# esteinig/sketchy

Hardware: AMD Instinct MI355X
Metric: reads/sec streamed (s=10000,k=16,40k-genome ref) (higher is better)
Workload: dtype u64

## Files before the change

sketchy_amd/csrc/skx_capi.hip:

```cpp
#include <dlfcn.h>
#include <hip/hip_runtime.h>
#include <rccl/rccl.h>

#include <unistd.h>

#include <algorithm>
#include <atomic>
#include <chrono>
#include <cmath>
#include <condition_variable>
#include <cstdarg>
#include <cstdio>
#include <cstdlib>
#include <cstring>
#include <mutex>
#include <string>
#include <thread>
#include <unordered_map>
#include <vector>

#include "sketchy_hip.h"
#include "skx_common.hpp"
#include "skx_kernels.hpp"

// ... 918 lines not shown
    hipEvent_t ev_pairq[2] = {nullptr, nullptr};
    bool pairq_pending[2] = {false, false};
    bool packed = false;
    u32 top_k = 0, max_reads = 0, sk_stride = 0;
    u64 max_bases = 0;
    u32 pcap = 0;
    u32 qcap = 0;
    u64* d_qd = nullptr;
    u32 *d_qrow = nullptr, *d_sslot = nullptr, *d_qinfo = nullptr, *d_qloc = nullptr, *d_cls_bsum = nullptr;
    u32* d_nd_hs = nullptr;
    u32* h_lcount = nullptr;
    u32 lcount_seq = 0, lcount_seen = 0, lcount_floor = 0;
    u32* h_nq_sink = nullptr;
    u32* h_nd = nullptr;
    u32 *d_rowcnt = nullptr;
    u32 *d_gain = nullptr;
    u32 *d_gain_s = nullptr;
    u32 *d_candslot = nullptr;
    u32 *d_candmask = nullptr;
    uint2 *d_lrow = nullptr;
    u32 *d_nlrow = nullptr, *d_gain_l = nullptr, *d_cbase = nullptr, *d_cwl = nullptr, *d_ncwl = nullptr;
    u64 *d_cw = nullptr;
    u64 *d_inb = nullptr, *d_hit = nullptr;
    skx::LongRows long_rows() const { return skx::LongRows{d_lrow, d_nlrow, qcap + 128, d_inb, ref->n_lw}; }
    bool use_pat = false;
    u32 *d_hist = nullptr, *d_nprow = nullptr;
    u64* d_pcw = nullptr;
    u32 npat_pad = 0;
    skx::PatRows pat_rows() const { return skx::PatRows{d_hist, npat_pad, d_gain_l, d_nprow}; }
    skx::RareIndex rare_index() const {
        skx::RareIndex ri = ref->rare_index();
        if (!use_pat) { ri.prec = nullptr; ri.n_pat = 0; }
        if (!static_dense) { ri.qs = nullptr; ri.n_sd = 0; }
        return ri;
    }
    u32 *d_cbad = nullptr, *d_nqc = nullptr;
    u32 *d_spc_g0 = nullptr, *d_spc_grp = nullptr;
    u32 n_pad_c = 0, n_grp_c = 0, cand_seq = 0;
    struct PassSet {
        u64 *tab = nullptr;
        u32 *cand = nullptr;
        u64 *tabc = nullptr;
        u32 *ncand = nullptr;
        u32 *mode = nullptr, *any_full = nullptr, *nqc_total = nullptr;
        u64 *mc = nullptr;
        u64 *mqc = nullptr;
        u64 *rowany_c = nullptr;
        u32 *grp_any_c = nullptr;
        u32 *smap = nullptr;
        u32 *pair_qc = nullptr;
        u32 *nd = nullptr;
        u32 *h_pub = nullptr;
    } ps[2];
    struct PassChains {
        bool pending = false, ranked = false, has_cand = false, update_table = false, forced_full = false, legacy = false;
        SubPass subs[kGroupMax];
        int n_sub = 0, b = 0, slot = 0;
        u32 P = 0, nq_rows = 0, seq = 0;
        u64 nq_est = 0;
// ... 646 lines not shown
        SCHK(hipMalloc(&st->d_cbad, 64));
        SCHK(hipMalloc(&st->d_nqc, skx::pass_counter_bytes()));
        std::vector<u32> g0c(n_sp), grpc(st->n_grp_c);
        for (u32 i = 0; i < n_sp; ++i) g0c[i] = i * cap;
        for (u32 i = 0; i < st->n_grp_c; ++i) grpc[i] = i / (cap / (skx::kRankWords * 64));
        SCHK(hipMalloc(&st->d_spc_g0, (size_t)n_sp * 4));
        SCHK(hipMalloc(&st->d_spc_grp, (size_t)st->n_grp_c * 4));
        SCHK(hipMemcpy(st->d_spc_g0, g0c.data(), (size_t)n_sp * 4, hipMemcpyHostToDevice));
        SCHK(hipMemcpy(st->d_spc_grp, grpc.data(), (size_t)st->n_grp_c * 4, hipMemcpyHostToDevice));
        for (auto& q : st->ps) {
            SCHK(hipMalloc(&q.tab, (size_t)(nb + 1) * n_pad * 8));
            SCHK(hipMalloc(&q.cand, (size_t)nb * st->n_pad_c * 4));
            SCHK(hipMalloc(&q.tabc, (size_t)nb * st->n_pad_c * 8));
            SCHK(hipMalloc(&q.ncand, (size_t)nb * n_sp * 4));
            SCHK(hipMalloc(&q.mode, 64)); SCHK(hipMalloc(&q.any_full, 64)); SCHK(hipMalloc(&q.nqc_total, 64));
            SCHK(hipMemset(q.any_full, 0, 64));
            SCHK(hipMalloc(&q.mc, (size_t)nb * (rows_c / 64) * st->n_pad_c * 8));
            SCHK(hipMalloc(&q.mqc, (size_t)nb * st->n_grp_c * rows_c * skx::kRankWords * 8));
            SCHK(hipMalloc(&q.rowany_c, (size_t)nb * st->n_grp_c * (rows_c / 64) * 8));
            SCHK(hipMalloc(&q.grp_any_c, (size_t)nb * st->n_grp_c * 4 + 64));
            SCHK(hipMalloc(&q.smap, (size_t)nb * ((size_t)st->qcap + 128) * 4));
            SCHK(hipMalloc(&q.pair_qc, (size_t)st->pcap * 4));
            SCHK(hipMalloc(&q.nd, 64));
            SCHK(hipMemset(q.nd, 0, 64));
            SCHK(hipHostMalloc((void**)&q.h_pub, 32 * 4, hipHostMallocCoherent));
            memset(q.h_pub, 0, 32 * 4);
        }
    }
    SCHK(hipDeviceSynchronize());
#undef SCHK
// ... 115 lines not shown
        const u32 any[4] = {skx::mq_any_stride(), 0xFFFFFFFFu, skx::mq_any_stride(), 0xFFFFFFFFu};
        e = hipMemcpy(st->d_mqext, any, sizeof(any), hipMemcpyHostToDevice);
    }
    if (e == hipSuccess && mint) e = hipMemset(mint, 0, (size_t)(rows / 64 + 2) * n_pad * 8);
    if (e == hipSuccess) e = hipDeviceSynchronize();
    if (e != hipSuccess) { undo(); return SKX_OK; }
    if (m) { (void)hipFree(st->d_m); st->d_m = m; }
    if (mint) { (void)hipFree(st->d_mint); st->d_mint = mint; }
    for (int i = 0; i < 2; ++i) {
        (void)hipFree(st->d_mq[i]); st->d_mq[i] = mq[i];
        (void)hipFree(st->d_rowany[i]); st->d_rowany[i] = ra[i];
        if (wb[i]) { (void)hipFree(st->d_wb[i]); st->d_wb[i] = wb[i]; }
        (void)hipFree(st->ps[i].smap); st->ps[i].smap = sm[i];
    }
    (void)hipFree(st->d_rowcnt); st->d_rowcnt = cnt;
    if (lrow) { (void)hipFree(st->d_lrow); st->d_lrow = lrow; }
    st->qcap = (u32)rows;
    st->mq_stride[0] = st->mq_stride[1] = 0;
    st->qrows_grown += 1;
    return SKX_OK;
}

static int queue_static_scan(skx_stream* st, int b) {
    if (!st->static_dense || st->m_ready[b]) return SKX_OK;
    const skx_ref* ref = st->ref;
    st->m_ready[b] = true;
    if (ref->n_sd == 0) return SKX_OK;
    if (st->reuse_m && st->m_filled[b]) return SKX_OK;
    st->m_filled[b] = true;
    static const bool big_slices = skx::knob("SKX_SCAN_BIGSLICE") && atoi(skx::knob("SKX_SCAN_BIGSLICE")) != 0;
// ... 158 lines not shown
    for (int i = 0; i < n_sub; ++i) pbt.p_off[i] = subs[i].p_off;
    pbt.p_off[n_sub] = P;
    auto rare_gains = [&](hipStream_t on) -> int {
        const skx::RareIndex ri = st->rare_index();
        const skx::LongRows lrows = st->long_rows();
        const skx::PatRows prows = st->pat_rows();
        skx::launch_gain_sparse(on, d_nd, q_bound, st->d_rowcnt, qstride, (u32)n_sub, n_pad, st->d_gain_s, st->d_sslot, ri, long_rows ? &lrows : nullptr, walk_scale,
                                (long_rows && st->use_pat) ? &prows : nullptr);
        if (long_rows) skx::launch_gain_long(on, lrows, ri, d_nd, st->d_rowcnt, qstride, (u32)n_sub, n_pad, st->d_gain_l, walk_scale);
        if (long_rows && st->use_pat)
            skx::launch_gain_dense(on, ri.pm, nullptr, n_pad, ri.d_npat, ri.n_pat, st->d_hist, st->npat_pad, (u32)n_sub, st->d_gain_l);
        HIPCHK(hipGetLastError());
        return SKX_OK;
    };
    auto row_counts = [&]() -> int {
        HIPCHK(hipMemset2DAsync(st->d_rowcnt, (size_t)qstride * 4, 0, (size_t)nq_rows * 4, (size_t)n_sub, hs));
        skx::launch_pass_hist(hs, d_pair_q, pbt, st->d_rowcnt, qstride);
        if (split_dict) HIPCHK(hipMemsetAsync(st->d_gain_s, 0, (size_t)n_sub * n_pad * 4 * skx::gain_sparse_stride(), hs));
        if (long_rows) {
            HIPCHK(hipMemsetAsync(st->d_nlrow, 0, skx::pass_counter_bytes(), hs));
            if (st->d_inb) {
                HIPCHK(hipMemsetAsync(st->d_inb, 0, (size_t)n_sub * ref->n_lw * 8, hs));
                HIPCHK(hipMemsetAsync(st->d_hit, 0, (size_t)n_sub * ref->n_lw * 8, hs));
            }
            HIPCHK(hipMemsetAsync(st->d_gain_l, 0, (size_t)n_sub * n_pad * 4, hs));
            if (st->use_pat) {
                HIPCHK(hipMemsetAsync(st->d_hist, 0, (size_t)n_sub * st->npat_pad * 4, hs));
                HIPCHK(hipMemsetAsync(st->d_nprow, 0, skx::pass_counter_bytes(), hs));
            }
        }
        return SKX_OK;
    };
    const u32 n_words = nq_rows / 64;
    bool split = false, lean_used = false;
    if (P > 0 && sdm) {
        st->total_passes += 1; st->lean_passes += 1;
        SKXCHK(wait_back());
    } else if (P > 0) {
        static const int split_env = skx::knob("SKX_SCAN_SPLIT") ? atoi(skx::knob("SKX_SCAN_SPLIT")) : -1;
        split = split_env >= 0 ? split_env != 0 : (nd_est * ref->rb / ref->s >= 192);
        if (split && !st->d_mint) {
            const size_t bytes = (size_t)(st->qcap / 64 + 2) * n_pad * 8;
            if (hipMalloc(&st->d_mint, bytes) == hipSuccess) {
                HIPCHK(hipMemsetAsync(st->d_mint, 0, bytes, hs));
            } else {
// ... 20 lines not shown
            Span sp(st, 1, hs);
            skx::launch_exceptions(hs, ref->d_exc_g, ref->d_exc_h, ref->n_exc, d_q, d_nq, d_m, n_pad, d_mdirty, split_dict ? st->d_qrow : nullptr);
        }
        SKXCHK(wait_back());
    }
    if (P == 0) SKXCHK(wait_back());

    if (update_table && !legacy && st->cum_writer) {
        HIPCHK(hipStreamWaitEvent(hs, st->cum_writer->ev_cum, 0));
        st->cum_writer = nullptr;
    }
    if (update_table && !legacy) {
        Span sp(st, 4, hs);
        const u32 n_sp = ref->n_species, cap = skx::kCandCap, rows_c = skx::kCandRows;
        const u64* m_int = split ? st->d_mint : nullptr;
        HIPCHK(hipMemsetAsync(st->d_gain, 0, (size_t)n_sub * n_pad * 4, hs));
        if (P > 0) {
            SKXCHK(row_counts());
            skx::launch_gain_dense(hs, d_m, m_int, n_pad, d_nd, sdm ? ref->n_sd : q_bound, st->d_rowcnt, qstride, (u32)n_sub, st->d_gain,
                                   (sdm && ref->n_species > 1) ? ref->d_segw : nullptr, ref->d_grp_sp);
            if (split_dict) SKXCHK(rare_gains(hs));
        }
        skx::launch_pass_tables(hs, st->d_cum, st->d_gain, (split_dict && P > 0) ? st->d_gain_s : nullptr,
                                (long_rows && P > 0) ? st->d_gain_l : nullptr, (u32)n_sub, n_pad, ps.tab);
        st->d_cum = ps.tab + (size_t)n_sub * n_pad;
        static const int cand_env = skx::knob("SKX_CAND") ? atoi(skx::knob("SKX_CAND")) : 1;
        static const int hint_env = skx::knob("SKX_CAND_HINT") ? atoi(skx::knob("SKX_CAND_HINT")) : 1;
        (void)hint_env;
        all_forced = !cand_env;
        u32 force_full = all_forced ? 0xFFu : 0u;
        for (int i = 0; i < n_sub; ++i) if (subs[i].d_shared || subs[i].d_counts) force_full |= 1u << i;
        HIPCHK(hipMemsetAsync(st->d_cbad, 0, 64, hs));
        HIPCHK(hipMemsetAsync(st->d_nqc, 0, skx::pass_counter_bytes(), hs));
        const bool pat_rows = st->use_pat && long_rows && ranked && P > 0 && !all_forced;
        if (pat_rows) skx::launch_pat_nqc_init(hs, st->d_nqc, st->npat_pad);
        if (ranked) {
            HIPCHK(hipMemsetAsync(st->d_candmask, 0, (size_t)n_pad * 4, hs));
            skx::launch_cand_select(hs, ps.tab, n_pad, spc, (u32)n_sub, st->top_k, cap, ps.cand, st->d_candslot, ps.tabc, ps.ncand, st->d_cbad,
                                    st->d_candmask);
            HIPCHK(hipMemsetAsync(ps.grp_any_c, 0, (size_t)n_sub * st->n_grp_c * 4, hs));
            if (split_dict && P > 0 && !all_forced) {
                HIPCHK(hipMemsetAsync(ps.mqc, 0, (size_t)n_sub * st->n_grp_c * rows_c * skx::kRankWords * 8, hs));
                HIPCHK(hipMemsetAsync(ps.rowany_c, 0, (size_t)n_sub * st->n_grp_c * (rows_c / 64) * 8, hs));
                HIPCHK(hipMemset2DAsync(ps.smap, (size_t)qstride * 4, 0, (size_t)nq_rows * 4, (size_t)n_sub, hs));
                skx::launch_cand_sparse(hs, st->d_sslot, d_nd, q_bound, st->rare_index(), st->d_candmask, st->d_candslot, n_pad, st->d_cbad, (u32)n_sub, st->d_nqc,
                                        ps.smap, qstride, ps.mqc, (size_t)st->n_grp_c * rows_c * skx::kRankWords, rows_c, ps.rowany_c,
                                        st->n_grp_c * (rows_c / 64), ps.grp_any_c, st->n_grp_c, walk_scale);
                if (long_rows) {
                    const u32 n_gw = n_pad / 64;
                    HIPCHK(hipMemsetAsync(st->d_cw, 0, (size_t)n_sub * n_gw * 8, hs));
                    HIPCHK(hipMemsetAsync(st->d_cbase, 0xFF, (size_t)n_sub * n_gw * 4, hs));
                    HIPCHK(hipMemsetAsync(st->d_ncwl, 0, 64, hs));
                    skx::launch_cand_words(hs, ps.cand, st->n_pad_c, (u32)n_sub, n_gw, st->d_cw, st->d_cbase, st->d_cwl, st->d_ncwl);
                    if (st->d_hit) skx::launch_cand_hit(hs, ps.cand, st->n_pad_c, (u32)n_sub, st->d_cbad, st->rare_index(), st->d_inb, st->d_hit);
                    skx::launch_cand_long(hs, st->long_rows(), st->rare_index(), d_nd, st->d_cw, st->d_cbase, st->d_cwl, st->d_ncwl, st->n_pad_c,
                                          st->d_cbad, (u32)n_sub, st->d_nqc, ps.smap, qstride, ps.mqc, (size_t)st->n_grp_c * rows_c * skx::kRankWords,
                                          rows_c, ps.rowany_c, st->n_grp_c * (rows_c / 64), ps.grp_any_c, st->n_grp_c, walk_scale, st->d_hit);
                }
                if (pat_rows) {
                    const skx::RareIndex ri = st->rare_index();
                    skx::launch_cand_pat_rows(hs, ri, d_nd, st->d_candmask, st->d_candslot, n_pad, st->d_cbad, (u32)n_sub, st->d_pcw, ps.mqc,
                                              (size_t)st->n_grp_c * rows_c * skx::kRankWords, rows_c, ps.rowany_c, st->n_grp_c * (rows_c / 64), ps.grp_any_c,
                                              st->n_grp_c);
                    skx::launch_cand_pat_map(hs, st->long_rows(), st->pat_rows(), ri, d_nd, st->d_candmask, st->d_candslot, n_pad, st->d_cbad, (u32)n_sub,
                                             st->d_nqc, ps.smap, qstride, st->d_pcw, ps.mqc, (size_t)st->n_grp_c * rows_c * skx::kRankWords, rows_c,
                                             ps.rowany_c, st->n_grp_c * (rows_c / 64), ps.grp_any_c, st->n_grp_c, q_bound, walk_scale);
                }
            }
        } else {
            HIPCHK(hipMemsetAsync(ps.ncand, 0, (size_t)n_sub * n_sp * 4, hs));
        }
        seq = ++st->cand_seq;
        skx::launch_cand_publish(hs, st->d_cbad, force_full, ps.ncand, st->d_nqc, d_nd, (u32)n_sub, n_sp, rows_c, ps.mode, ps.any_full,
                                 ps.nqc_total, ps.h_pub, seq);
        if (ranked && P > 0 && !all_forced)
            skx::launch_cand_gather_m(hs, d_m, m_int, n_pad, d_nd, sdm ? ref->n_sd : q_bound, ps.cand, st->n_pad_c, st->d_cbad, (u32)n_sub, ps.mc, rows_c / 64);
        only_if = ps.any_full;
        HIPCHK(hipGetLastError());
    }
    if (P > 0) {
        static const int direct_env = skx::knob("SKX_RARE_DIRECT") ? atoi(skx::knob("SKX_RARE_DIRECT")) : 1;
        const bool direct_rare = split_dict && ref->rare_direct && (direct_env != 0 || sdm);
        if (split_dict && !direct_rare) {
            Span sp(st, 1, hs);
            skx::launch_sparse_fill(hs, st->d_sslot, d_nd, st->rare_index(), d_m, n_pad, d_mdirty, q_bound, only_if);
        }
        if (!direct_rare) HIPCHK(hipMemsetAsync(st->d_mqext + 2 * b, 0, 8, hs));
        {
            Span sp(st, 3, hs);
// ... 1484 lines not shown
    SKXCHK(flush_pending(st));
    HIPCHK(hipStreamSynchronize(st->hs0));
    HIPCHK(hipStreamSynchronize(st->hs1));
    HIPCHK(hipStreamSynchronize(st->hs));
    HIPCHK(hipMemsetAsync(st->d_cum, 0, (size_t)st->ref->n_pad * 8, st->hs2));
    if (st->d_seen) HIPCHK(hipMemsetAsync(st->d_seen, 0, (size_t)st->seen_words * 4, st->hs2));
    HIPCHK(hipStreamSynchronize(st->hs2));
    st->reads_total = 0;
    st->h_nq[2] = 1; st->h_nq[3] = 1;
    st->hint_all_overflow = false;
    st->hint_seq = st->cand_seq;
    st->legacy_run = 0;
    st->lcount_floor = st->lcount_seq;
    st->fresh_table = true;
    st->cum_writer = nullptr;
    return SKX_OK;
}
SKX_API int skx_stream_reads(const skx_stream* st, uint64_t* n_reads) {
    if (!st || !n_reads) return fail(SKX_ERR_INVALID, "NULL argument");
    *n_reads = st->reads_total;
    for (int i = 0; i < st->n_pend; ++i) *n_reads += st->pend[i].n_reads;
    return SKX_OK;
}
SKX_API int skx_stream_stats(skx_stream* st, uint64_t* out, uint32_t n_out) {
    if (!st || !out) return fail(SKX_ERR_INVALID, "NULL argument");
    uint64_t live = 0;
    SKXCHK(use_device(st->device));
    SKXCHK(skx_stream_sync(st));
    {
        const u32 n_grp = st->ref->n_pad / (skx::kRankWords * 64);
// ... 946 lines not shown
```

sketchy_amd/csrc/skx_kernels.hip:

```cpp
#include <algorithm>
#include <cstdlib>
#include <mutex>
#include <type_traits>

#include "skx_common.hpp"
#include "skx_kernels.hpp"

#ifndef SKX_FEW_CANDS
#define SKX_FEW_CANDS 8
#endif
#ifndef SKX_SCAN_ROWS
#define SKX_SCAN_ROWS 8
#endif
#ifndef SKX_SCAN_OCC
#define SKX_SCAN_OCC 1
#endif
#ifndef SKX_SCAN_SPLIT_READS
#define SKX_SCAN_SPLIT_READS 1
#endif
#ifndef SKX_WALK_BLOCKS
#define SKX_WALK_BLOCKS 256
#endif
#ifndef SKX_GAIN_SPARSE_STRIDE
#define SKX_GAIN_SPARSE_STRIDE 16
// ... 4032 lines not shown
                    atomicOr(&rowany_c[(size_t)b * rowany_stride + (size_t)grp * (rows_c >> 6) + (cr >> 6)], 1ull << (cr & 63u));
                    u32* ga = grp_any_c + (size_t)b * n_grp_c + grp;
                    if (*ga == 0u) atomicOr(ga, 1u);
                }
            }
            wave_sync();
        } else {
            for (u32 grp = lane; grp < n_grp_c; grp += 64u) {
                atomicOr(&rowany_c[(size_t)b * rowany_stride + (size_t)grp * (rows_c >> 6) + (cr >> 6)], 1ull << (cr & 63u));
                u32* ga = grp_any_c + (size_t)b * n_grp_c + grp;
                if (*ga == 0u) atomicOr(ga, 1u);
            }
        }
    }
}
__global__ void pat_nqc_init_kernel(u32* __restrict__ nqc, u32 v) {
    if (threadIdx.x < kPassBatchesMax) nqc[threadIdx.x * kCtrStride] = v;
}
__global__ __launch_bounds__(256) void cand_pat_rows_kernel(RareIndex ri, const u32* __restrict__ n_d, const u32* __restrict__ candmask,
                                                            const u32* __restrict__ candslot, u32 n_pad, u32* __restrict__ bad,
                                                            u64* __restrict__ pcw, u64* __restrict__ mqc, size_t mqc_stride, u32 rows_c,
                                                            u64* __restrict__ rowany_c, u32 rowany_stride, u32* __restrict__ grp_any_c,
                                                            u32 n_grp_c) {
    __builtin_amdgcn_s_setprio(2);
    __shared__ u64 pat[4][kPatWords];
    const u32 b = blockIdx.y, lane = lane_id(), wv = threadIdx.x >> 6, p = blockIdx.x * 4u + wv;
    if (p >= ri.n_pat || bad[b]) return;
    const u32 nd64 = n_d[2], n_gw_c = n_grp_c * kRankWords, npat64 = (ri.n_pat + 63u) & ~63u;
    if (nd64 + npat64 + 64u >= rows_c) { if (lane == 0u) atomicOr(&bad[b], 2u); return; }
    const u32 cr = nd64 + p;
    u64* pw = pat[wv];
    for (u32 w = lane; w < n_gw_c; w += 64u) pw[w] = 0ull;
// ... 347 lines not shown
                        hit &= ~__ballot(mine && (s_ >> 6) / kRankWords == grp);
                        if (!((fl >> (grp & 63u)) & 1ull) || grp >= 64u) {
                            if (lane == l0) flag(b, cr, grp);
                            fl |= 1ull << (grp & 63u);
                        }
                    }
#pragma unroll
                    for (u32 i = 0; i < kPassBatchesMax; ++i) if (i == b) { crow[i] = cr; flagged[i] = fl; }
                }
            }
        }
    }
}
__global__ void cand_publish_kernel(const u32* __restrict__ bad, u32 force_full, const u32* __restrict__ ncand, const u32* __restrict__ nqc,
                                    const u32* __restrict__ n_d, u32 n_b, u32 n_sp, u32 rows_c, u32* __restrict__ mode, u32* __restrict__ any_full,
                                    u32* __restrict__ nqc_total, volatile u32* __restrict__ h_pub, u32 seq) {
    __builtin_amdgcn_s_setprio(3);
    if (threadIdx.x != 0 || blockIdx.x != 0) return;
    u32 any = 0;
    const u32 nd64 = n_d[2];
    for (u32 b = 0; b < n_b; ++b) {
        const bool full = bad[b] != 0u || ((force_full >> b) & 1u) || nd64 + 64u >= rows_c;
        mode[b] = full ? 0u : 1u;
        any |= full ? 1u : 0u;
        u32 mx = 0;
        for (u32 s_ = 0; s_ < n_sp; ++s_) mx = max(mx, ncand[b * n_sp + s_]);
        nqc_total[b] = nd64 + nqc[b * kCtrStride];
        h_pub[b] = full ? 0u : 1u;
        h_pub[kPassBatchesMax + b] = mx;
    }
    *any_full = any;
    h_pub[2 * kPassBatchesMax] = any;
    h_pub[2 * kPassBatchesMax + 2] = n_b;
    __threadfence_system();
    h_pub[2 * kPassBatchesMax + 1] = seq;
    __threadfence_system();
}
__global__ __launch_bounds__(256) void m_clear_kernel(u64* __restrict__ m_bits, u64* __restrict__ m_int, u32 n_pad,
                                                      const u32* __restrict__ n_d, const u32* __restrict__ any_full) {
    if (*any_full) return;
    const u32 n_words = (n_d[0] + 63u) >> 6;
    const size_t n = (size_t)n_words * n_pad;
// ... 372 lines not shown
}
void launch_list_sig(hipStream_t st, const u32* lslot, u32 n_long, const u32* off, const u32* cnt, const u32* post, u32* sig, u64* content) {
    if (n_long == 0) return;
    hipLaunchKernelGGL(list_sig_kernel, dim3(cdiv(n_long, 4)), dim3(256), 0, st, lslot, n_long, off, cnt, post, sig, content);
}
void launch_pat_exceptions(hipStream_t st, const u64* mlong, u32 n_gw, u32 n_long, const u32* pat_of, const u32* pat_rep, u32* prec, u32* n_done) {
    if (n_long == 0) return;
    hipLaunchKernelGGL(pat_exceptions_kernel, dim3(cdiv(n_long, 4)), dim3(256), 0, st, mlong, n_gw, n_long, pat_of, pat_rep, prec, n_done);
}
void launch_pat_matrix(hipStream_t st, const u64* mlong, const u32* pat_rep, u32 n_pat, u32 n_gw, u64* pm, u32 n_pad) {
    if (n_pat == 0) return;
    hipLaunchKernelGGL(pat_matrix_kernel, dim3(cdiv(n_pat, 64), cdiv(n_gw, 4)), dim3(256), 0, st, mlong, pat_rep, n_pat, n_gw, pm, n_pad);
}
u32 pat_record_words() { return kPatRec; }
u32 pat_words_max() { return kPatWords; }
void launch_pat_nqc_init(hipStream_t st, u32* nqc, u32 v) { hipLaunchKernelGGL(pat_nqc_init_kernel, dim3(1), dim3(64), 0, st, nqc, v); }
void launch_cand_pat_rows(hipStream_t st, const RareIndex& ri, const u32* n_d, const u32* candmask, const u32* candslot, u32 n_pad, u32* bad, u32 n_b,
                          u64* pcw, u64* mqc, size_t mqc_stride, u32 rows_c, u64* rowany_c, u32 rowany_stride, u32* grp_any_c, u32 n_grp_c) {
    if (ri.n_pat == 0) return;
    hipLaunchKernelGGL(cand_pat_rows_kernel, dim3(cdiv(ri.n_pat, 4), n_b), dim3(256), 0, st, ri, n_d, candmask, candslot, n_pad, bad, pcw, mqc, mqc_stride,
                       rows_c, rowany_c, rowany_stride, grp_any_c, n_grp_c);
}
void launch_cand_pat_map(hipStream_t st, const LongRows& lr, const PatRows& pr, const RareIndex& ri, const u32* n_d, const u32* candmask,
                         const u32* candslot, u32 n_pad, u32* bad, u32 n_b, u32* nqc, u32* smap, u32 smap_stride, const u64* pcw, u64* mqc,
                         size_t mqc_stride, u32 rows_c, u64* rowany_c, u32 rowany_stride, u32* grp_any_c, u32 n_grp_c, u32 rows_bound, u32 walk_scale) {
    const u32 blocks = std::max(1u, std::min(cdiv(rows_bound, 256), 64u * std::max(1u, walk_scale)));
    hipLaunchKernelGGL(cand_pat_map_kernel, dim3(blocks, n_b), dim3(256), 0, st, lr, pr, ri, n_d, candmask, candslot, n_pad, bad, nqc, smap, smap_stride,
                       pcw, mqc, mqc_stride, rows_c, rowany_c, rowany_stride, grp_any_c, n_grp_c);
}
u32 gain_sparse_stride() { return kGainSparseStride; }
u32 pass_counter_bytes() { return kPassBatchesMax * kCtrStride * 4u; }
// ... 34 lines not shown
void launch_cand_count(hipStream_t st, const u64* t0, const u64* t1, const Species& sp, u32 top_k, u32* h_out, u32 seq) {
    hipLaunchKernelGGL(cand_count_kernel, dim3(1), dim3(1024), 0, st, t0, t1, sp, top_k, nullptr, h_out, seq);
}
void launch_cand_gather_m(hipStream_t st, const u64* m_bits, const u64* m_int, u32 n_pad, const u32* n_d, u32 rows_bound, const u32* cand, u32 n_pad_c,
                          const u32* bad, u32 n_b, u64* mc, u32 words_c) {
    const u32 words = std::min(words_c, std::max(1u, cdiv(rows_bound, 64)));
    hipLaunchKernelGGL(cand_gather_m_kernel, dim3(cdiv(n_pad_c, 256), words, n_b), dim3(256), 0, st, m_bits, m_int, n_pad, n_d, cand, n_pad_c, bad, mc, words_c);
}
void launch_cand_sparse(hipStream_t st, const u32* sslot, const u32* n_d, u32 rows_bound, const RareIndex& ri, const u32* candmask,
                        const u32* candslot, u32 n_pad, u32* bad, u32 n_b, u32* nqc, u32* smap, u32 smap_stride, u64* mqc, size_t mqc_stride,
                        u32 rows_c, u64* rowany_c, u32 rowany_stride, u32* grp_any_c, u32 n_grp_c, u32 walk_scale) {
    hipLaunchKernelGGL(cand_sparse_kernel, dim3(std::max(1u, std::min(cdiv(rows_bound, 256), kWalkBlocks * std::max(1u, walk_scale)))), dim3(256), 0, st, sslot, n_d, ri, candmask,
                       candslot, n_pad, bad, n_b, nqc, smap, smap_stride, mqc, mqc_stride, rows_c, rowany_c, rowany_stride, grp_any_c, n_grp_c);
}
void launch_cand_publish(hipStream_t st, const u32* bad, u32 force_full, const u32* ncand, const u32* nqc, const u32* n_d, u32 n_b, u32 n_sp,
                         u32 rows_c, u32* mode, u32* any_full, u32* nqc_total, u32* h_pub, u32 seq) {
    hipLaunchKernelGGL(cand_publish_kernel, dim3(1), dim3(1), 0, st, bad, force_full, ncand, nqc, n_d, n_b, n_sp, rows_c, mode, any_full, nqc_total,
                       h_pub, seq);
}
void launch_m_clear(hipStream_t st, u64* m_bits, u64* m_int, u32 n_pad, const u32* n_d, const u32* any_full) {
    hipLaunchKernelGGL(m_clear_kernel, dim3(512), dim3(256), 0, st, m_bits, m_int, n_pad, n_d, any_full);
}
void launch_cand_pair_rows(hipStream_t st, const u32* pair_q, u32 n_pairs, const u32* n_d, const u32* smap, u32 rows_c, u32* pair_qc) {
    if (n_pairs == 0) return;
    hipLaunchKernelGGL(cand_pair_rows_kernel, dim3(cdiv(n_pairs, 256)), dim3(256), 0, st, pair_q, n_pairs, n_d, smap, rows_c, pair_qc);
}
void launch_cand_rows_back(hipStream_t st, u32* out_idx, u32 n_reads, u32 n_sp, u32 top_k, const u32* cand, u32 cap, const u32* g0) {
    const u32 n = n_reads * n_sp * top_k;
    if (n == 0) return;
    hipLaunchKernelGGL(cand_rows_back_kernel, dim3(cdiv(n, 256)), dim3(256), 0, st, out_idx, n, n_sp, top_k, cand, cap, g0);
}
template <int KMAX, bool EXACT>
static void consensus_rows_go(hipStream_t st, const u32* idx, u32 n_out, u32 n_sp, u32 top_k, const u32* g0, const u32* codes, u32 n_code_rows,
// ... 690 lines not shown
```

sketchy_amd/csrc/skx_kernels.hpp:

```cpp
#pragma once
#include <hip/hip_runtime.h>
#include <stddef.h>
#include <stdint.h>

#include <stdlib.h>

namespace skx {
typedef unsigned long long u64;
typedef unsigned int u32;

inline const char* knob(const char* name) {
#ifdef SKX_EXPERIMENTS
    return getenv(name);
#else
    (void)name;
    return nullptr;
#endif
}

constexpr int kSketchCap = 2048;
constexpr u32 kSegLen = 64;
constexpr int kRankWords = 8;

struct Species { const u32* g0; const u32* n; const u32* of_grp; u32 n_sp; };
// ... 62 lines not shown
                       u64* spmask = nullptr , const u32* grp_sp = nullptr, u32 s = 0);
void launch_rare_fill(hipStream_t st, const u64* mat, u64 n_elems, u32 s, const u64* key, const u32* off, u32* cursor, u32* post, u32 mask);
void launch_classify(hipStream_t st, const u64* q, const u32* n_q, u32 q_bound, const RareIndex& ri, u32* qinfo, u32* qloc, u32* bsum,
                     u64* qd, u32* n_d, u32* qrow, u32* sslot, u32* h_words);
void launch_rare_to_mq(hipStream_t st, const u32* sslot, const u32* n_d, const RareIndex& ri, u64* mq, u32 nq_rows, u32 n_pad, u64* rowany,
                       u32* grp_any, u32 rows_bound, const u32* only_if, u32* ext);
u32 mq_any_stride();
void launch_sparse_fill(hipStream_t st, const u32* sslot, const u32* n_d, const RareIndex& ri, u64* m_bits, u32 n_pad, u32* m_dirty,
                        u32 rows_bound, const u32* only_if = nullptr );
void launch_nd_from_nq(hipStream_t st, const u32* n_q, u32* n_d, u32* h_words);

static const u32 kPassBatchesMax = 8;
static const u32 kCandCap = 1024;
static const u32 kCandRows = 131072;
struct PassBatches { u32 n; u32 p_off[kPassBatchesMax + 1]; };
void launch_pass_hist(hipStream_t st, const u32* pair_q, const PassBatches& pb, u32* cnt, u32 row_stride);
void launch_gain_dense(hipStream_t st, const u64* m_bits, const u64* m_int , u32 n_pad, const u32* n_d, u32 rows_bound, const u32* cnt,
                       u32 row_stride, u32 n_b, u32* gain, const u32* segw = nullptr ,
                       const u32* grp_sp = nullptr);
void launch_gain_sparse(hipStream_t st, const u32* n_d, u32 rows_bound, const u32* cnt, u32 row_stride, u32 n_b, u32 n_pad, u32* gain_s,
                        const u32* sslot, const RareIndex& ri, const LongRows* lr, u32 walk_scale, const PatRows* pr = nullptr);
void launch_pat_nqc_init(hipStream_t st, u32* nqc, u32 v);
void launch_cand_pat_rows(hipStream_t st, const RareIndex& ri, const u32* n_d, const u32* candmask, const u32* candslot, u32 n_pad, u32* bad, u32 n_b,
                          u64* pcw, u64* mqc, size_t mqc_stride, u32 rows_c, u64* rowany_c, u32 rowany_stride, u32* grp_any_c, u32 n_grp_c);
void launch_cand_pat_map(hipStream_t st, const LongRows& lr, const PatRows& pr, const RareIndex& ri, const u32* n_d, const u32* candmask,
                         const u32* candslot, u32 n_pad, u32* bad, u32 n_b, u32* nqc, u32* smap, u32 smap_stride, const u64* pcw, u64* mqc,
                         size_t mqc_stride, u32 rows_c, u64* rowany_c, u32 rowany_stride, u32* grp_any_c, u32 n_grp_c, u32 rows_bound, u32 walk_scale = 1);
u32 gain_sparse_stride();
void launch_pass_tables(hipStream_t st, const u64* prev, const u32* gain, const u32* gain_s , const u32* gain_l , u32 n_b,
                        u32 n_pad, u64* tab);
void launch_cand_select(hipStream_t st, const u64* tab, u32 n_pad, const Species& sp, u32 n_b, u32 top_k, u32 cap, u32* cand, u32* candslot,
                        u64* tabc, u32* ncand, u32* bad, u32* candmask);
void launch_cand_count(hipStream_t st, const u64* t0, const u64* t1, const Species& sp, u32 top_k, u32* h_out, u32 seq);
void launch_cand_gather_m(hipStream_t st, const u64* m_bits, const u64* m_int , u32 n_pad, const u32* n_d, u32 rows_bound, const u32* cand,
                          u32 n_pad_c, const u32* bad, u32 n_b, u64* mc, u32 words_c);
void launch_cand_sparse(hipStream_t st, const u32* sslot, const u32* n_d, u32 rows_bound, const RareIndex& ri, const u32* candmask,
                        const u32* candslot, u32 n_pad, u32* bad, u32 n_b, u32* nqc, u32* smap, u32 smap_stride, u64* mqc, size_t mqc_stride,
                        u32 rows_c, u64* rowany_c, u32 rowany_stride, u32* grp_any_c, u32 n_grp_c, u32 walk_scale = 1);
void launch_cand_publish(hipStream_t st, const u32* bad, u32 force_full, const u32* ncand, const u32* nqc, const u32* n_d, u32 n_b, u32 n_sp,
                         u32 rows_c, u32* mode, u32* any_full, u32* nqc_total, u32* h_pub, u32 seq);
void launch_m_clear(hipStream_t st, u64* m_bits, u64* m_int , u32 n_pad, const u32* n_d, const u32* any_full);
void launch_cand_pair_rows(hipStream_t st, const u32* pair_q, u32 n_pairs, const u32* n_d, const u32* smap, u32 rows_c, u32* pair_qc);
void launch_cand_rows_back(hipStream_t st, u32* out_idx, u32 n_reads, u32 n_sp, u32 top_k, const u32* cand, u32 cap, const u32* g0);
constexpr u32 kConsensusTopMax = 64;
void launch_consensus_rows(hipStream_t st, const u32* idx, u64 first_row, u64 n_rows, u32 n_sp, u32 top_k, const u32* g0, const u32* codes,
                           u32 n_feat, u32* out, u32 n_code_rows);
constexpr u32 kChangeWidthMax = 4096;
void launch_change_flags(hipStream_t st, const u32* rows, u32 width, u32 ra, u32 rb, u32* flag);
void launch_change_events(hipStream_t st, const u32* flag, u32* pos, u32* bsum, u32 n, u32 cap, u32* n_events, u32* ev_read,
                          const u32* idx, const u64* sum, u32 w_idx, u32* ev_idx, u64* ev_sum, const u32* codes, u32 w_codes, u32* ev_codes);
void launch_species_call(hipStream_t st, const u32* idx, const u64* sum, const u32* codes, u32 ra, u32 rb, u32 n_sp, u32 top_k, u32 n_feat,
                         u32* call_sp, u32* call_idx, u64* call_sum, u32* call_codes, u32* key, bool key_codes);
void launch_call_species_gather(hipStream_t st, const u32* flag, const u32* pos, u32 n, u32 cap, const u32* call_sp, u32* ev_sp);

void launch_pair_q(hipStream_t st, const u64* pair_h, u32 n_pairs, const u64* q, const u32* n_q, u32* pair_q, const u32* qrow ,
// ... 112 lines not shown
```

Baseline: 147.2 million.

## Batch per-pass buffer clears into one kernel and bound clears by used extents

Replaces a dozen-plus hipMemsetAsync/hipMemset2DAsync calls in the candidate front-end with a single pass_clear kernel that clears a table of ranges. It also records how many rows of mqc/rowany_c/smap/rowcnt the previous pass actually wrote, via a new ext output from cand_publish and host-side slot extents, so later clears only zero the dirty prefix instead of whole buffers. This cuts launch overhead and memset bandwidth per pass. The cost is extra bookkeeping with whole-buffer fallbacks on reset or regrow, and a risk of stale data if an extent is underestimated.

```diff
diff --git a/sketchy_amd/csrc/skx_capi.hip b/sketchy_amd/csrc/skx_capi.hip
--- a/sketchy_amd/csrc/skx_capi.hip
+++ b/sketchy_amd/csrc/skx_capi.hip
@@ -956,6 +956,9 @@
     u32* h_nq_sink = nullptr;
     u32* h_nd = nullptr;
     u32 *d_rowcnt = nullptr;
+    skx::SlotExtents rowcnt_ext;
+    bool front_open = false;
+    void extents_unknown() { rowcnt_ext.whole(); for (auto& q : ps) { q.smap_ext.whole(); q.mqc_whole = 0xFFu; } }
     u32 *d_gain = nullptr;
     u32 *d_gain_s = nullptr;
     u32 *d_candslot = nullptr;
@@ -985,6 +988,9 @@
         u64 *tabc = nullptr;
         u32 *ncand = nullptr;
         u32 *mode = nullptr, *any_full = nullptr, *nqc_total = nullptr;
+        u32 *ext = nullptr;
+        skx::SlotExtents smap_ext;
+        u32 mqc_whole = 0xFFu;
         u64 *mc = nullptr;
         u64 *mqc = nullptr;
         u64 *rowany_c = nullptr;
@@ -1661,6 +1667,7 @@
             SCHK(hipMalloc(&q.tabc, (size_t)nb * st->n_pad_c * 8));
             SCHK(hipMalloc(&q.ncand, (size_t)nb * n_sp * 4));
             SCHK(hipMalloc(&q.mode, 64)); SCHK(hipMalloc(&q.any_full, 64)); SCHK(hipMalloc(&q.nqc_total, 64));
+            q.ext = q.nqc_total + skx::kPassBatchesMax;
             SCHK(hipMemset(q.any_full, 0, 64));
             SCHK(hipMalloc(&q.mc, (size_t)nb * (rows_c / 64) * st->n_pad_c * 8));
             SCHK(hipMalloc(&q.mqc, (size_t)nb * st->n_grp_c * rows_c * skx::kRankWords * 8));
@@ -1806,6 +1813,8 @@
         (void)hipFree(st->ps[i].smap); st->ps[i].smap = sm[i];
     }
     (void)hipFree(st->d_rowcnt); st->d_rowcnt = cnt;
+    st->rowcnt_ext.whole();
+    for (auto& q : st->ps) q.smap_ext.whole();
     if (lrow) { (void)hipFree(st->d_lrow); st->d_lrow = lrow; }
     st->qcap = (u32)rows;
     st->mq_stride[0] = st->mq_stride[1] = 0;
@@ -1994,21 +2003,7 @@
         return SKX_OK;
     };
     auto row_counts = [&]() -> int {
-        HIPCHK(hipMemset2DAsync(st->d_rowcnt, (size_t)qstride * 4, 0, (size_t)nq_rows * 4, (size_t)n_sub, hs));
         skx::launch_pass_hist(hs, d_pair_q, pbt, st->d_rowcnt, qstride);
-        if (split_dict) HIPCHK(hipMemsetAsync(st->d_gain_s, 0, (size_t)n_sub * n_pad * 4 * skx::gain_sparse_stride(), hs));
-        if (long_rows) {
-            HIPCHK(hipMemsetAsync(st->d_nlrow, 0, skx::pass_counter_bytes(), hs));
-            if (st->d_inb) {
-                HIPCHK(hipMemsetAsync(st->d_inb, 0, (size_t)n_sub * ref->n_lw * 8, hs));
-                HIPCHK(hipMemsetAsync(st->d_hit, 0, (size_t)n_sub * ref->n_lw * 8, hs));
-            }
-            HIPCHK(hipMemsetAsync(st->d_gain_l, 0, (size_t)n_sub * n_pad * 4, hs));
-            if (st->use_pat) {
-                HIPCHK(hipMemsetAsync(st->d_hist, 0, (size_t)n_sub * st->npat_pad * 4, hs));
-                HIPCHK(hipMemsetAsync(st->d_nprow, 0, skx::pass_counter_bytes(), hs));
-            }
-        }
         return SKX_OK;
     };
     const u32 n_words = nq_rows / 64;
@@ -2059,43 +2054,78 @@
         Span sp(st, 4, hs);
         const u32 n_sp = ref->n_species, cap = skx::kCandCap, rows_c = skx::kCandRows;
         const u64* m_int = split ? st->d_mint : nullptr;
-        HIPCHK(hipMemsetAsync(st->d_gain, 0, (size_t)n_sub * n_pad * 4, hs));
-        if (P > 0) {
-            SKXCHK(row_counts());
-            skx::launch_gain_dense(hs, d_m, m_int, n_pad, d_nd, sdm ? ref->n_sd : q_bound, st->d_rowcnt, qstride, (u32)n_sub, st->d_gain,
-                                   (sdm && ref->n_species > 1) ? ref->d_segw : nullptr, ref->d_grp_sp);
-            if (split_dict) SKXCHK(rare_gains(hs));
-        }
-        skx::launch_pass_tables(hs, st->d_cum, st->d_gain, (split_dict && P > 0) ? st->d_gain_s : nullptr,
-                                (long_rows && P > 0) ? st->d_gain_l : nullptr, (u32)n_sub, n_pad, ps.tab);
-        st->d_cum = ps.tab + (size_t)n_sub * n_pad;
         static const int cand_env = skx::knob("SKX_CAND") ? atoi(skx::knob("SKX_CAND")) : 1;
         static const int hint_env = skx::knob("SKX_CAND_HINT") ? atoi(skx::knob("SKX_CAND_HINT")) : 1;
         (void)hint_env;
         all_forced = !cand_env;
         u32 force_full = all_forced ? 0xFFu : 0u;
         for (int i = 0; i < n_sub; ++i) if (subs[i].d_shared || subs[i].d_counts) force_full |= 1u << i;
-        HIPCHK(hipMemsetAsync(st->d_cbad, 0, 64, hs));
-        HIPCHK(hipMemsetAsync(st->d_nqc, 0, skx::pass_counter_bytes(), hs));
         const bool pat_rows = st->use_pat && long_rows && ranked && P > 0 && !all_forced;
-        if (pat_rows) skx::launch_pat_nqc_init(hs, st->d_nqc, st->npat_pad);
+        const bool fill_mqc = ranked && split_dict && P > 0 && !all_forced;
+        const u32 n_gw = n_pad / 64;
+        {
+            if (st->front_open) st->extents_unknown();
+            st->front_open = true;
+            skx::PassClear pcl;
+            bool ok = skx::clear_add(pcl, st->d_gain, (size_t)n_sub * n_pad * 4);
+            if (P > 0) {
+                ok = ok && skx::clear_add_slots(pcl, st->d_rowcnt, qstride, st->rowcnt_ext, (u32)n_sub);
+                st->rowcnt_ext.used((u32)n_sub, nq_rows);
+                if (split_dict) ok = ok && skx::clear_add(pcl, st->d_gain_s, (size_t)n_sub * n_pad * 4 * skx::gain_sparse_stride());
+                if (long_rows) {
+                    ok = ok && skx::clear_add(pcl, st->d_nlrow, skx::pass_counter_bytes());
+                    if (st->d_inb) {
+                        ok = ok && skx::clear_add(pcl, st->d_inb, (size_t)n_sub * ref->n_lw * 8);
+                        ok = ok && skx::clear_add(pcl, st->d_hit, (size_t)n_sub * ref->n_lw * 8);
+                    }
+                    ok = ok && skx::clear_add(pcl, st->d_gain_l, (size_t)n_sub * n_pad * 4);
+                    if (st->use_pat) {
+                        ok = ok && skx::clear_add(pcl, st->d_hist, (size_t)n_sub * st->npat_pad * 4);
+                        ok = ok && skx::clear_add(pcl, st->d_nprow, skx::pass_counter_bytes());
+                    }
+                }
+            }
+            ok = ok && skx::clear_add(pcl, st->d_cbad, 64);
+            pcl.nqc = st->d_nqc; pcl.nqc_words = skx::pass_counter_bytes() / 4; pcl.nqc_stride = skx::pass_counter_stride();
+            pcl.nqc_start = pat_rows ? st->npat_pad : 0u;
+            if (ranked) {
+                ok = ok && skx::clear_add(pcl, st->d_candmask, (size_t)n_pad * 4);
+                ok = ok && skx::clear_add(pcl, ps.grp_any_c, (size_t)n_sub * st->n_grp_c * 4);
+                if (fill_mqc) {
+                    pcl.mqc = ps.mqc; pcl.rowany_c = ps.rowany_c; pcl.ext = ps.ext;
+                    pcl.n_b = (u32)n_sub; pcl.n_grp_c = st->n_grp_c; pcl.rows_c = rows_c; pcl.whole_mask = ps.mqc_whole;
+                    ps.mqc_whole &= ~((1u << n_sub) - 1u);
+                    ok = ok && skx::clear_add_slots(pcl, ps.smap, qstride, ps.smap_ext, (u32)n_sub);
+                    ps.smap_ext.used((u32)n_sub, nq_rows);
+                    if (long_rows) {
+                        ok = ok && skx::clear_add(pcl, st->d_cw, (size_t)n_sub * n_gw * 8);
+                        ok = ok && skx::clear_add(pcl, st->d_cbase, (size_t)n_sub * n_gw * 4, 0xFFu);
+                        ok = ok && skx::clear_add(pcl, st->d_ncwl, 64);
+                    }
+                }
+            } else {
+                ok = ok && skx::clear_add(pcl, ps.ncand, (size_t)n_sub * n_sp * 4);
+            }
+            if (!ok) return fail(SKX_ERR_HIP, "internal: the pass's clear table is full or a range is not word-aligned");
+            skx::launch_pass_clear(hs, pcl);
+        }
+        if (P > 0) {
+            SKXCHK(row_counts());
+            skx::launch_gain_dense(hs, d_m, m_int, n_pad, d_nd, sdm ? ref->n_sd : q_bound, st->d_rowcnt, qstride, (u32)n_sub, st->d_gain,
+                                   (sdm && ref->n_species > 1) ? ref->d_segw : nullptr, ref->d_grp_sp);
+            if (split_dict) SKXCHK(rare_gains(hs));
+        }
+        skx::launch_pass_tables(hs, st->d_cum, st->d_gain, (split_dict && P > 0) ? st->d_gain_s : nullptr,
+                                (long_rows && P > 0) ? st->d_gain_l : nullptr, (u32)n_sub, n_pad, ps.tab);
+        st->d_cum = ps.tab + (size_t)n_sub * n_pad;
         if (ranked) {
-            HIPCHK(hipMemsetAsync(st->d_candmask, 0, (size_t)n_pad * 4, hs));
             skx::launch_cand_select(hs, ps.tab, n_pad, spc, (u32)n_sub, st->top_k, cap, ps.cand, st->d_candslot, ps.tabc, ps.ncand, st->d_cbad,
                                     st->d_candmask);
-            HIPCHK(hipMemsetAsync(ps.grp_any_c, 0, (size_t)n_sub * st->n_grp_c * 4, hs));
-            if (split_dict && P > 0 && !all_forced) {
-                HIPCHK(hipMemsetAsync(ps.mqc, 0, (size_t)n_sub * st->n_grp_c * rows_c * skx::kRankWords * 8, hs));
-                HIPCHK(hipMemsetAsync(ps.rowany_c, 0, (size_t)n_sub * st->n_grp_c * (rows_c / 64) * 8, hs));
-                HIPCHK(hipMemset2DAsync(ps.smap, (size_t)qstride * 4, 0, (size_t)nq_rows * 4, (size_t)n_sub, hs));
+            if (fill_mqc) {
                 skx::launch_cand_sparse(hs, st->d_sslot, d_nd, q_bound, st->rare_index(), st->d_candmask, st->d_candslot, n_pad, st->d_cbad, (u32)n_sub, st->d_nqc,
                                         ps.smap, qstride, ps.mqc, (size_t)st->n_grp_c * rows_c * skx::kRankWords, rows_c, ps.rowany_c,
                                         st->n_grp_c * (rows_c / 64), ps.grp_any_c, st->n_grp_c, walk_scale);
                 if (long_rows) {
-                    const u32 n_gw = n_pad / 64;
-                    HIPCHK(hipMemsetAsync(st->d_cw, 0, (size_t)n_sub * n_gw * 8, hs));
-                    HIPCHK(hipMemsetAsync(st->d_cbase, 0xFF, (size_t)n_sub * n_gw * 4, hs));
-                    HIPCHK(hipMemsetAsync(st->d_ncwl, 0, 64, hs));
                     skx::launch_cand_words(hs, ps.cand, st->n_pad_c, (u32)n_sub, n_gw, st->d_cw, st->d_cbase, st->d_cwl, st->d_ncwl);
                     if (st->d_hit) skx::launch_cand_hit(hs, ps.cand, st->n_pad_c, (u32)n_sub, st->d_cbad, st->rare_index(), st->d_inb, st->d_hit);
                     skx::launch_cand_long(hs, st->long_rows(), st->rare_index(), d_nd, st->d_cw, st->d_cbase, st->d_cwl, st->d_ncwl, st->n_pad_c,
@@ -2112,12 +2142,11 @@
                                              ps.rowany_c, st->n_grp_c * (rows_c / 64), ps.grp_any_c, st->n_grp_c, q_bound, walk_scale);
                 }
             }
-        } else {
-            HIPCHK(hipMemsetAsync(ps.ncand, 0, (size_t)n_sub * n_sp * 4, hs));
         }
         seq = ++st->cand_seq;
         skx::launch_cand_publish(hs, st->d_cbad, force_full, ps.ncand, st->d_nqc, d_nd, (u32)n_sub, n_sp, rows_c, ps.mode, ps.any_full,
-                                 ps.nqc_total, ps.h_pub, seq);
+                                 ps.nqc_total, ps.h_pub, seq, fill_mqc ? ps.ext : nullptr);
+        st->front_open = false;
         if (ranked && P > 0 && !all_forced)
             skx::launch_cand_gather_m(hs, d_m, m_int, n_pad, d_nd, sdm ? ref->n_sd : q_bound, ps.cand, st->n_pad_c, st->d_cbad, (u32)n_sub, ps.mc, rows_c / 64);
         only_if = ps.any_full;
@@ -3632,6 +3661,7 @@
     st->lcount_floor = st->lcount_seq;
     st->fresh_table = true;
     st->cum_writer = nullptr;
+    st->extents_unknown();
     return SKX_OK;
 }
 SKX_API int skx_stream_reads(const skx_stream* st, uint64_t* n_reads) {
diff --git a/sketchy_amd/csrc/skx_kernels.hip b/sketchy_amd/csrc/skx_kernels.hip
--- a/sketchy_amd/csrc/skx_kernels.hip
+++ b/sketchy_amd/csrc/skx_kernels.hip
@@ -4070,8 +4070,31 @@
         }
     }
 }
-__global__ void pat_nqc_init_kernel(u32* __restrict__ nqc, u32 v) {
-    if (threadIdx.x < kPassBatchesMax) nqc[threadIdx.x * kCtrStride] = v;
+
+__device__ __forceinline__ void fill_words(u32* __restrict__ p, u64 n, u32 v, u64 tid, u64 n_thr) {
+    const u64 head = min(n, (u64)(((16u - (u32)((size_t)p & 15u)) & 15u) >> 2));
+    if (tid < head) p[tid] = v;
+    uint4* q = reinterpret_cast<uint4*>(p + head);
+    const u64 nv = (n - head) >> 2, tail = (n - head) & 3ull;
+    const uint4 vv = make_uint4(v, v, v, v);
+    for (u64 i = tid; i < nv; i += n_thr) q[i] = vv;
+    if (tid < tail) p[head + nv * 4ull + tid] = v;
+}
+__global__ __launch_bounds__(256) void pass_clear_kernel(PassClear pc) {
+    const u64 tid = (u64)blockIdx.x * 256u + threadIdx.x, n_thr = (u64)gridDim.x * 256u;
+    for (u32 k = 0; k < pc.n; ++k) fill_words(static_cast<u32*>(pc.r[k].p), pc.r[k].bytes >> 2, pc.r[k].fill ? 0xFFFFFFFFu : 0u, tid, n_thr);
+    if (pc.nqc && tid < pc.nqc_words) pc.nqc[tid] = (tid % pc.nqc_stride == 0ull) ? pc.nqc_start : 0u;
+    if (pc.mqc) {
+        const u32 rows_c = pc.rows_c;
+        for (u32 i = 0; i < pc.n_b; ++i) {
+            const u32 e = ((pc.whole_mask >> i) & 1u) ? rows_c : min(pc.ext[i], rows_c);
+            for (u32 grp = 0; grp < pc.n_grp_c; ++grp) {
+                const size_t at = (size_t)i * pc.n_grp_c + grp;
+                fill_words(reinterpret_cast<u32*>(pc.mqc + at * rows_c * kRankWords), (u64)e * kRankWords * 2u, 0u, tid, n_thr);
+                fill_words(reinterpret_cast<u32*>(pc.rowany_c + at * (rows_c >> 6)), (u64)((e + 63u) >> 6) * 2u, 0u, tid, n_thr);
+            }
+        }
+    }
 }
 __global__ __launch_bounds__(256) void cand_pat_rows_kernel(RareIndex ri, const u32* __restrict__ n_d, const u32* __restrict__ candmask,
                                                             const u32* __restrict__ candslot, u32 n_pad, u32* __restrict__ bad,
@@ -4449,7 +4472,7 @@
 }
 __global__ void cand_publish_kernel(const u32* __restrict__ bad, u32 force_full, const u32* __restrict__ ncand, const u32* __restrict__ nqc,
                                     const u32* __restrict__ n_d, u32 n_b, u32 n_sp, u32 rows_c, u32* __restrict__ mode, u32* __restrict__ any_full,
-                                    u32* __restrict__ nqc_total, volatile u32* __restrict__ h_pub, u32 seq) {
+                                    u32* __restrict__ nqc_total, volatile u32* __restrict__ h_pub, u32 seq, u32* __restrict__ ext) {
     __builtin_amdgcn_s_setprio(3);
     if (threadIdx.x != 0 || blockIdx.x != 0) return;
     u32 any = 0;
@@ -4461,6 +4484,7 @@
         u32 mx = 0;
         for (u32 s_ = 0; s_ < n_sp; ++s_) mx = max(mx, ncand[b * n_sp + s_]);
         nqc_total[b] = nd64 + nqc[b * kCtrStride];
+        if (ext) ext[b] = bad[b] != 0u ? rows_c : min(rows_c, nd64 + nqc[b * kCtrStride]);
         h_pub[b] = full ? 0u : 1u;
         h_pub[kPassBatchesMax + b] = mx;
     }
@@ -4863,7 +4887,13 @@
 }
 u32 pat_record_words() { return kPatRec; }
 u32 pat_words_max() { return kPatWords; }
-void launch_pat_nqc_init(hipStream_t st, u32* nqc, u32 v) { hipLaunchKernelGGL(pat_nqc_init_kernel, dim3(1), dim3(64), 0, st, nqc, v); }
+void launch_pass_clear(hipStream_t st, const PassClear& pc) {
+    u64 bytes = pc.mqc ? (u64)pc.n_b * pc.n_grp_c * 4096u * 64u : 0u;
+    for (u32 k = 0; k < pc.n; ++k) bytes += pc.r[k].bytes;
+    const u32 blocks = (u32)std::min<u64>(1024u, std::max<u64>(16u, bytes / (256u * 64u)));
+    hipLaunchKernelGGL(pass_clear_kernel, dim3(blocks), dim3(256), 0, st, pc);
+}
+u32 pass_counter_stride() { return kCtrStride; }
 void launch_cand_pat_rows(hipStream_t st, const RareIndex& ri, const u32* n_d, const u32* candmask, const u32* candslot, u32 n_pad, u32* bad, u32 n_b,
                           u64* pcw, u64* mqc, size_t mqc_stride, u32 rows_c, u64* rowany_c, u32 rowany_stride, u32* grp_any_c, u32 n_grp_c) {
     if (ri.n_pat == 0) return;
@@ -4928,9 +4958,9 @@
                        candslot, n_pad, bad, n_b, nqc, smap, smap_stride, mqc, mqc_stride, rows_c, rowany_c, rowany_stride, grp_any_c, n_grp_c);
 }
 void launch_cand_publish(hipStream_t st, const u32* bad, u32 force_full, const u32* ncand, const u32* nqc, const u32* n_d, u32 n_b, u32 n_sp,
-                         u32 rows_c, u32* mode, u32* any_full, u32* nqc_total, u32* h_pub, u32 seq) {
+                         u32 rows_c, u32* mode, u32* any_full, u32* nqc_total, u32* h_pub, u32 seq, u32* ext) {
     hipLaunchKernelGGL(cand_publish_kernel, dim3(1), dim3(1), 0, st, bad, force_full, ncand, nqc, n_d, n_b, n_sp, rows_c, mode, any_full, nqc_total,
-                       h_pub, seq);
+                       h_pub, seq, ext);
 }
 void launch_m_clear(hipStream_t st, u64* m_bits, u64* m_int, u32 n_pad, const u32* n_d, const u32* any_full) {
     hipLaunchKernelGGL(m_clear_kernel, dim3(512), dim3(256), 0, st, m_bits, m_int, n_pad, n_d, any_full);
diff --git a/sketchy_amd/csrc/skx_kernels.hpp b/sketchy_amd/csrc/skx_kernels.hpp
--- a/sketchy_amd/csrc/skx_kernels.hpp
+++ b/sketchy_amd/csrc/skx_kernels.hpp
@@ -4,6 +4,8 @@
 #include <stdint.h>
 
 #include <stdlib.h>
+
+#include "skx_pass_clear.hpp"
 
 namespace skx {
 typedef unsigned long long u64;
@@ -100,13 +102,15 @@
 static const u32 kCandCap = 1024;
 static const u32 kCandRows = 131072;
 struct PassBatches { u32 n; u32 p_off[kPassBatchesMax + 1]; };
+static_assert(kClearSlotsMax == kPassBatchesMax, "one extent per batch slot");
+void launch_pass_clear(hipStream_t st, const PassClear& pc);
+u32 pass_counter_stride();
 void launch_pass_hist(hipStream_t st, const u32* pair_q, const PassBatches& pb, u32* cnt, u32 row_stride);
 void launch_gain_dense(hipStream_t st, const u64* m_bits, const u64* m_int , u32 n_pad, const u32* n_d, u32 rows_bound, const u32* cnt,
                        u32 row_stride, u32 n_b, u32* gain, const u32* segw = nullptr ,
                        const u32* grp_sp = nullptr);
 void launch_gain_sparse(hipStream_t st, const u32* n_d, u32 rows_bound, const u32* cnt, u32 row_stride, u32 n_b, u32 n_pad, u32* gain_s,
                         const u32* sslot, const RareIndex& ri, const LongRows* lr, u32 walk_scale, const PatRows* pr = nullptr);
-void launch_pat_nqc_init(hipStream_t st, u32* nqc, u32 v);
 void launch_cand_pat_rows(hipStream_t st, const RareIndex& ri, const u32* n_d, const u32* candmask, const u32* candslot, u32 n_pad, u32* bad, u32 n_b,
                           u64* pcw, u64* mqc, size_t mqc_stride, u32 rows_c, u64* rowany_c, u32 rowany_stride, u32* grp_any_c, u32 n_grp_c);
 void launch_cand_pat_map(hipStream_t st, const LongRows& lr, const PatRows& pr, const RareIndex& ri, const u32* n_d, const u32* candmask,
@@ -124,7 +128,8 @@
                         const u32* candslot, u32 n_pad, u32* bad, u32 n_b, u32* nqc, u32* smap, u32 smap_stride, u64* mqc, size_t mqc_stride,
                         u32 rows_c, u64* rowany_c, u32 rowany_stride, u32* grp_any_c, u32 n_grp_c, u32 walk_scale = 1);
 void launch_cand_publish(hipStream_t st, const u32* bad, u32 force_full, const u32* ncand, const u32* nqc, const u32* n_d, u32 n_b, u32 n_sp,
-                         u32 rows_c, u32* mode, u32* any_full, u32* nqc_total, u32* h_pub, u32 seq);
+                         u32 rows_c, u32* mode, u32* any_full, u32* nqc_total, u32* h_pub, u32 seq,
+                         u32* ext = nullptr );
 void launch_m_clear(hipStream_t st, u64* m_bits, u64* m_int , u32 n_pad, const u32* n_d, const u32* any_full);
 void launch_cand_pair_rows(hipStream_t st, const u32* pair_q, u32 n_pairs, const u32* n_d, const u32* smap, u32 rows_c, u32* pair_qc);
 void launch_cand_rows_back(hipStream_t st, u32* out_idx, u32 n_reads, u32 n_sp, u32 top_k, const u32* cand, u32 cap, const u32* g0);
diff --git a/sketchy_amd/csrc/skx_pass_clear.hpp b/sketchy_amd/csrc/skx_pass_clear.hpp
--- /dev/null
+++ b/sketchy_amd/csrc/skx_pass_clear.hpp
@@ -0,0 +1,48 @@
+#pragma once
+#include <stddef.h>
+#include <stdint.h>
+
+namespace skx {
+
+constexpr unsigned kClearRangesMax = 40;
+constexpr unsigned kClearSlotsMax = 8;
+constexpr unsigned kExtentWhole = 0xFFFFFFFFu;
+
+struct ClearRange {
+    void* p;
+    unsigned long long bytes;
+    unsigned fill;
+};
+struct PassClear {
+    unsigned n = 0;
+    ClearRange r[kClearRangesMax];
+    unsigned* nqc = nullptr;
+    unsigned nqc_words = 0, nqc_stride = 1, nqc_start = 0;
+    unsigned long long* mqc = nullptr;
+    unsigned long long* rowany_c = nullptr;
+    const unsigned* ext = nullptr;
+    unsigned n_b = 0, n_grp_c = 0, rows_c = 0, whole_mask = 0;
+};
+
+inline bool clear_add(PassClear& pc, void* p, size_t bytes, unsigned fill = 0u) {
+    if (bytes == 0) return true;
+    if (pc.n >= kClearRangesMax || (bytes & 3u) || ((uintptr_t)p & 3u)) return false;
+    pc.r[pc.n++] = ClearRange{p, (unsigned long long)bytes, fill};
+    return true;
+}
+
+struct SlotExtents {
+    unsigned rows[kClearSlotsMax];
+    SlotExtents() { whole(); }
+    void whole() { for (unsigned i = 0; i < kClearSlotsMax; ++i) rows[i] = kExtentWhole; }
+    void used(unsigned n_b, unsigned nq_rows) { for (unsigned i = 0; i < n_b && i < kClearSlotsMax; ++i) rows[i] = nq_rows; }
+};
+inline bool clear_add_slots(PassClear& pc, unsigned* base, size_t stride, const SlotExtents& ext, unsigned n_b) {
+    for (unsigned i = 0; i < n_b && i < kClearSlotsMax; ++i) {
+        const size_t rows = ext.rows[i] < stride ? ext.rows[i] : stride;
+        if (!clear_add(pc, base + (size_t)i * stride, rows * 4u)) return false;
+    }
+    return true;
+}
+
+}
```

After: 153.1 million (median of 6 runs). 1.04x the previous value.
